# yongjianxu/ompi-release

Measured on AMD Instinct MI355X. Metric: MPI_Allreduce busbw GB/s (1 GiB fp32, np=8) + op/hip reduce HBM GB/s, higher is better.
Workload: dtype f32; 1 GPU; op/hip 3-buff MPI_SUM MPI_FLOAT, 1 GiB per operand (BASELINE configs[1]); count=268435456, bytes_per_operand=1073741824

## Files before the change

### include/mi355x_rt.h

```cpp
#ifndef MI355X_RT_H
#define MI355X_RT_H

#include <stddef.h>
#include <stdint.h>

#include "mi355x_types.h"

#ifdef __cplusplus
extern "C" {
#endif

const char *mi355x_last_error(void);
int mi355x_version(void);
int mi355x_device_count(int *count);
int mi355x_set_device(int dev);
int mi355x_get_device(int *dev);
int mi355x_stream_create(void **stream);
int mi355x_stream_destroy(void *stream);
int mi355x_stream_sync(void *stream);
int mi355x_device_sync(void);
int mi355x_malloc(void **p, size_t bytes);
int mi355x_free(void *p);
int mi355x_host_alloc(void **p, size_t bytes);
int mi355x_host_free(void *p);
// ... 31 lines not shown
int mi355x_comm_rank(const mi355x_comm_t *comm);
int mi355x_comm_size(const mi355x_comm_t *comm);
int mi355x_comm_barrier(mi355x_comm_t *comm);
int mi355x_comm_vote(mi355x_comm_t *comm, int device, int *engine);
int mi355x_comm_last_algorithm(const mi355x_comm_t *comm);
int mi355x_debug_pipe_token(mi355x_comm_t *comm, int acquire);
int mi355x_debug_token(uint64_t dev_uid, const char *name, int op);

enum mi355x_knob {
    MI355X_KNOB_ALLREDUCE_ALG = 1,
    MI355X_KNOB_REDUCE_ALG = 2,
    MI355X_KNOB_REDUCE_SCATTER_ALG = 3,
    MI355X_KNOB_BLOCKS_PER_CU = 4,
    MI355X_KNOB_TIMEOUT_S = 5,
    MI355X_KNOB_PUSH = 6,
    MI355X_KNOB_IPC_MAX_BYTES = 7,
    MI355X_KNOB_STAGE_BYTES = 8,
    MI355X_KNOB_REDUCE_CHAIN_FANOUT = 10,
    MI355X_KNOB_LL_MAX_BYTES = 9,
    MI355X_KNOB_TIME_PHASES = 11,
    MI355X_KNOB_COPY_BLOCK_KIB = 12,
    MI355X_KNOB_PIPE = 13,
    MI355X_KNOB_PIPE_WG_PER_CU = 14,
    MI355X_KNOB_PIPE_CHUNK_KIB = 15,
    MI355X_KNOB_PIPE_WT = 16,
    MI355X_KNOB_ONE_PHASE_MAX_BYTES = 17,
    MI355X_KNOB_PIPE_REFUSED = 18,
    MI355X_KNOB_SVC_MAX_BYTES = 19,
    MI355X_KNOB_SVC_CALLS = 20,
    MI355X_KNOB_SVC_LAUNCHES = 21,
    MI355X_KNOB_SVC_RESIDENT = 22,
    MI355X_KNOB_SVC_PULL_MAX_BYTES = 23,
    MI355X_KNOB_SVC_PULL_COPY_MAX_BYTES = 24,
    MI355X_KNOB_RCACHE_MAX_MAPS = 25,
    MI355X_KNOB_RCACHE_SIZE_LIMIT = 26,
    MI355X_KNOB_PEER_MAPS = 27,
    MI355X_KNOB_RCACHE_EVICTIONS = 28,
    MI355X_KNOB_FLOWS = 29,
    MI355X_KNOB_FLOWS_FAILED = 30,
    MI355X_KNOB_CREATE_US = 31,
    MI355X_KNOB_SELFTEST_US = 32,
    MI355X_KNOB_SVC_OWNER = 33,
    MI355X_KNOB_SVC_CLAIMS = 34,
    MI355X_KNOB_SVC_IDLE_US = 35,
    MI355X_KNOB_SVC_SHRINK_US = 36,
    MI355X_KNOB_SVC_REGROWS = 37,
    MI355X_KNOB_DEV_SETUP = 38,
    MI355X_KNOB_SETUP_US = 39,
    MI355X_KNOB_SELFTEST = 40,
    MI355X_KNOB_PIPE_CALLS = 41,
    MI355X_KNOB_EXPORT_MISMATCHES = 42,
    MI355X_KNOB_SELFTEST_REUSED = 43,
    MI355X_KNOB_NB_ORDER = 44,
    MI355X_KNOB_SCAN_PART_MIN_BYTES = 45
};
enum mi355x_flow {
    MI355X_FLOW_SVC_LL = 1,
    MI355X_FLOW_SVC_PULL = 2,
    MI355X_FLOW_SVC_COPY = 4,
    MI355X_FLOW_SVC_RS = 8,
    MI355X_FLOW_PIPE = 16
};
int mi355x_comm_set(mi355x_comm_t *comm, int knob, long value);
int mi355x_comm_get(const mi355x_comm_t *comm, int knob, long *value);
int mi355x_comm_phase_ms(const mi355x_comm_t *comm, float *phase1_ms, float *phase2_ms);

enum mi355x_coll_id {
    MI355X_COLL_ALLGATHER = 0, MI355X_COLL_ALLREDUCE = 2, MI355X_COLL_BCAST = 7, MI355X_COLL_REDUCE = 11,
    MI355X_COLL_REDUCESCATTER = 12, MI355X_COLL_COUNT = 16
};
typedef struct mi355x_rules mi355x_rules_t;
int mi355x_rules_load(const char *path, mi355x_rules_t **rules);
int mi355x_rules_destroy(mi355x_rules_t *rules);
int mi355x_rules_decide(const mi355x_rules_t *rules, int coll, int comm_size, size_t msg_bytes, int *alg,
                        int *faninout, int *segsize);
int mi355x_comm_set_rules(mi355x_comm_t *comm, const mi355x_rules_t *rules);

int mi355x_allreduce(mi355x_comm_t *comm, const void *sbuf, void *rbuf, size_t count, int type, int op,
                     void *stream);
int mi355x_reduce(mi355x_comm_t *comm, const void *sbuf, void *rbuf, size_t count, int type, int op, int root,
                  void *stream);
int mi355x_reduce_scatter_block(mi355x_comm_t *comm, const void *sbuf, void *rbuf, size_t rcount,
                                int type, int op, void *stream);
int mi355x_reduce_scatter(mi355x_comm_t *comm, const void *sbuf, void *rbuf, const int *rcounts,
                          int type, int op, void *stream);
int mi355x_allgather(mi355x_comm_t *comm, const void *sbuf, void *rbuf, size_t bytes, void *stream);
int mi355x_bcast(mi355x_comm_t *comm, void *buf, size_t bytes, int root, void *stream);

int mi355x_gather(mi355x_comm_t *comm, const void *sbuf, void *rbuf, size_t bytes, int root, void *stream);
int mi355x_gatherv(mi355x_comm_t *comm, const void *sbuf, size_t sbytes, void *rbuf, const size_t *rcounts,
                   const size_t *displs, int root, void *stream);
int mi355x_scatter(mi355x_comm_t *comm, const void *sbuf, void *rbuf, size_t bytes, int root, void *stream);
int mi355x_scatterv(mi355x_comm_t *comm, const void *sbuf, const size_t *scounts, const size_t *displs,
                    void *rbuf, size_t rbytes, int root, void *stream);
int mi355x_allgatherv(mi355x_comm_t *comm, const void *sbuf, size_t sbytes, void *rbuf, const size_t *rcounts,
                      const size_t *displs, void *stream);
int mi355x_alltoall(mi355x_comm_t *comm, const void *sbuf, void *rbuf, size_t bytes, void *stream);
int mi355x_alltoallv(mi355x_comm_t *comm, const void *sbuf, const size_t *scounts, const size_t *sdispls,
                     void *rbuf, const size_t *rcounts, const size_t *rdispls, void *stream);
int mi355x_scan(mi355x_comm_t *comm, const void *sbuf, void *rbuf, size_t count, int type, int op, void *stream);
int mi355x_exscan(mi355x_comm_t *comm, const void *sbuf, void *rbuf, size_t count, int type, int op, void *stream);
int mi355x_scan_part_plan(size_t count, int n, int q, int r, size_t *src_off, size_t *len, size_t *slot_off);

typedef struct mi355x_request mi355x_request_t;
int mi355x_iallreduce(mi355x_comm_t *comm, const void *sbuf, void *rbuf, size_t count, int type, int op,
                      void *stream, mi355x_request_t **req);
// ... 89 lines not shown
```

### ompi-release_amd/__init__.py

```python
from __future__ import annotations

import ctypes
import os
import pathlib

PKG_DIR = pathlib.Path(__file__).resolve().parent
LIB_DIR = pathlib.Path(os.environ["MI355X_LIB_DIR"]) if os.environ.get("MI355X_LIB_DIR") else PKG_DIR / "lib"
REPO_DIR = PKG_DIR.parent

TYPES = [
    "INT8", "UINT8", "INT16", "UINT16", "INT32", "UINT32", "INT64", "UINT64",
    "F_INTEGER", "F_INTEGER1", "F_INTEGER2", "F_INTEGER4", "F_INTEGER8", "F_INTEGER16",
    "FLOAT", "DOUBLE", "F_REAL", "F_REAL2", "F_REAL4", "F_REAL8", "F_REAL16",
    "F_DOUBLE_PRECISION", "LONG_DOUBLE", "F_LOGICAL", "BOOL",
    "C_FLOAT_COMPLEX", "C_DOUBLE_COMPLEX", "C_LONG_DOUBLE_COMPLEX", "BYTE",
    "F_2REAL", "F_2DOUBLE_PRECISION", "F_2INTEGER",
    "FLOAT_INT", "DOUBLE_INT", "LONG_INT", "2INT", "SHORT_INT", "LONG_DOUBLE_INT", "WCHAR",
]
T = {name: i for i, name in enumerate(TYPES)}
OPS = ["NULL", "MAX", "MIN", "SUM", "PROD", "LAND", "BAND", "LOR", "BOR", "LXOR", "BXOR",
       "MAXLOC", "MINLOC", "REPLACE", "NO_OP"]
OP = {name: i for i, name in enumerate(OPS)}

MI355X_SUCCESS = 0
# ... 181 lines not shown

def op_supported(op: int, ty: int) -> bool:
    return bool(rt().mi355x_op_supported(op, ty))


def comm_op_supported(op: int, ty: int) -> bool:
    return bool(rt().mi355x_comm_op_supported(op, ty))


def type_size(ty: int) -> int:
    return int(rt().mi355x_type_size(ty))


def set_threads(threads: int) -> None:
    check(rt().mi355x_op_set_threads(threads), "mi355x_op_set_threads")


def tune(unroll: int = 0, blocks_per_cu: int = 0, nontemporal: int = -2) -> None:
    check(rt().mi355x_op_tune(unroll, blocks_per_cu, nontemporal), "mi355x_op_tune")


def set_mode(mode: int) -> None:
    check(rt().mi355x_op_set_mode(mode), "mi355x_op_set_mode")


def get_mode() -> int:
    return int(rt().mi355x_op_get_mode())


def get_tune() -> tuple[int, int, int]:
    a, b, c = ctypes.c_int(), ctypes.c_int(), ctypes.c_int()
    check(rt().mi355x_op_get_tune(ctypes.byref(a), ctypes.byref(b), ctypes.byref(c)))
    return a.value, b.value, c.value


def scan_part_plan(count: int, n: int, q: int, r: int) -> tuple[int, int, int | None]:
    a, b, c_ = ctypes.c_size_t(), ctypes.c_size_t(), ctypes.c_size_t()
    check(rt().mi355x_scan_part_plan(count, n, q, r, ctypes.byref(a), ctypes.byref(b), ctypes.byref(c_)),
          "mi355x_scan_part_plan")
    return a.value, b.value, None if r == q else c_.value


KNOB = {"ALLREDUCE_ALG": 1, "REDUCE_ALG": 2, "REDUCE_SCATTER_ALG": 3, "BLOCKS_PER_CU": 4, "TIMEOUT_S": 5,
        "PUSH": 6, "IPC_MAX_BYTES": 7, "STAGE_BYTES": 8,
        "LL_MAX_BYTES": 9, "REDUCE_CHAIN_FANOUT": 10, "TIME_PHASES": 11,
        "COPY_BLOCK_KIB": 12, "PIPE": 13, "PIPE_WG_PER_CU": 14, "PIPE_CHUNK_KIB": 15, "PIPE_WT": 16,
        "ONE_PHASE_MAX_BYTES": 17, "PIPE_REFUSED": 18, "SVC_MAX_BYTES": 19, "SVC_CALLS": 20,
        "SVC_LAUNCHES": 21, "SVC_RESIDENT": 22, "SVC_PULL_MAX_BYTES": 23,
        "SVC_PULL_COPY_MAX_BYTES": 24, "RCACHE_MAX_MAPS": 25, "RCACHE_SIZE_LIMIT": 26, "PEER_MAPS": 27,
        "RCACHE_EVICTIONS": 28, "FLOWS": 29, "FLOWS_FAILED": 30, "CREATE_US": 31, "SELFTEST_US": 32,
        "SVC_OWNER": 33, "SVC_CLAIMS": 34, "SVC_IDLE_US": 35,
        "SVC_SHRINK_US": 36, "SVC_REGROWS": 37, "DEV_SETUP": 38, "SETUP_US": 39, "SELFTEST": 40,
        "PIPE_CALLS": 41, "EXPORT_MISMATCHES": 42, "SELFTEST_REUSED": 43, "NB_ORDER": 44,
        "SCAN_PART_MIN_BYTES": 45}
NBC_ALG = {"BINOMIAL": 101, "RING": 102, "CHAIN": 103}
FLOW = {"SVC_LL": 1, "SVC_PULL": 2, "SVC_COPY": 4, "SVC_RS": 8, "PIPE": 16}
COLL = {"ALLGATHER": 0, "ALLREDUCE": 2, "BCAST": 7, "REDUCE": 11, "REDUCESCATTER": 12}
AR_ALG = {"DECISION": 0, "LINEAR": 1, "NONOVERLAPPING": 2, "RECURSIVE_DOUBLING": 3, "RING": 4,
          "RING_SEGMENTED": 5}


class Comm:

    def __init__(self, handle: int):
        self.h = ctypes.c_void_p(handle)

    @classmethod
    def create(cls, key: str, rank: int, size: int, device: int) -> "Comm":
        h = ctypes.c_void_p()
        check(rt().mi355x_comm_create(key.encode(), rank, size, device, ctypes.byref(h)), "mi355x_comm_create")
        return cls(h.value)

    @classmethod
    def loopback(cls, size: int, device: int = 0) -> list["Comm"]:
        arr = (ctypes.c_void_p * size)()
        check(rt().mi355x_comm_create_loopback(size, device, arr), "mi355x_comm_create_loopback")
        return [cls(arr[i]) for i in range(size)]

    def destroy(self) -> None:
        if self.h:
            rt().mi355x_comm_destroy(self.h)
            self.h = ctypes.c_void_p()

    @property
    def rank(self) -> int:
        return rt().mi355x_comm_rank(self.h)

    @property
    def size(self) -> int:
        return rt().mi355x_comm_size(self.h)

    def barrier(self) -> None:
        check(rt().mi355x_comm_barrier(self.h), "mi355x_comm_barrier")

    def vote(self, device: bool) -> bool:
        anyd = ctypes.c_int(0)
        check(rt().mi355x_comm_vote(self.h, 1 if device else 0, ctypes.byref(anyd)), "mi355x_comm_vote")
        return bool(anyd.value)

    def last_algorithm(self) -> int:
        return rt().mi355x_comm_last_algorithm(self.h)

    def debug_pipe_token(self, acquire: bool) -> bool:
        rc = rt().mi355x_debug_pipe_token(self.h, 1 if acquire else 0)
        if rc < 0:
            check(rc, "mi355x_debug_pipe_token")
        return rc == 1
# ... 336 lines not shown
```

### ompi-release_amd/csrc/rt/coll_comm.cpp

```cpp

#include <fcntl.h>
#include <immintrin.h>
#include <poll.h>
#include <sched.h>
#include <signal.h>
#include <sys/mman.h>
#include <sys/socket.h>
#include <sys/stat.h>
#include <sys/un.h>
#include <unistd.h>

#include <algorithm>
#include <array>
#include <atomic>
#include <cerrno>
#include <chrono>
#include <condition_variable>
#include <cstddef>
#include <deque>
#include <functional>
#include <cstdio>
#include <cstdlib>
#include <cstring>
#include <map>
// ... 326 lines not shown
    if (op) return (c->pipe_entry >= 0 || pipe_token_acquire(c)) ? 1 : 0;
    if (c->pipe_entry >= 0) pipe_token_release(c);
    return 0;
}

int mi355x_debug_pipe_token(mi355x_comm_t *c, int acquire)
{
    if (!c) return set_error(MI355X_ERR_ARG, "comm is NULL");
    if (acquire) return pipe_token_acquire(c) ? 1 : 0;
    if (c->pipe_entry >= 0) pipe_token_release(c);
    return 0;
}
static bool svc_limit_visible(const mi355x_comm_t *c)
{
    return c->svc_ok || c->svc_want || (!c->dev_ready && !c->loopback && c->size > 1);
}

int mi355x_comm_get(const mi355x_comm_t *c, int knob, long *value)
{
    if (!c || !value) return set_error(MI355X_ERR_ARG, "NULL argument");
    switch (knob) {
    case MI355X_KNOB_ALLREDUCE_ALG: *value = c->knob_allreduce; break;
    case MI355X_KNOB_REDUCE_ALG: *value = c->knob_reduce; break;
    case MI355X_KNOB_REDUCE_SCATTER_ALG: *value = c->knob_rs; break;
    case MI355X_KNOB_BLOCKS_PER_CU: *value = c->tune.blocks_per_cu; break;
    case MI355X_KNOB_TIMEOUT_S: *value = (long)c->timeout_s; break;
    case MI355X_KNOB_PUSH: *value = c->tune.push; break;
    case MI355X_KNOB_IPC_MAX_BYTES: *value = (long)c->ipc_max; break;
    case MI355X_KNOB_STAGE_BYTES: *value = (long)c->stage_bytes; break;
    case MI355X_KNOB_PIPE_REFUSED: *value = (long)c->pipe_refused; break;
    case MI355X_KNOB_LL_MAX_BYTES: *value = (long)c->ll_max; break;
    case MI355X_KNOB_REDUCE_CHAIN_FANOUT: *value = c->chain_fanout; break;
    case MI355X_KNOB_TIME_PHASES: *value = c->time_phases ? 1 : 0; break;
    case MI355X_KNOB_COPY_BLOCK_KIB: *value = c->tune.copy_block_kib; break;
    case MI355X_KNOB_PIPE: *value = c->pipe_on ? 1 : 0; break;
    case MI355X_KNOB_PIPE_WG_PER_CU: *value = c->tune.pipe_wg_per_cu; break;
    case MI355X_KNOB_PIPE_CHUNK_KIB: *value = c->tune.pipe_chunk_kib; break;
    case MI355X_KNOB_PIPE_WT: *value = c->tune.pipe_wt; break;
    case MI355X_KNOB_ONE_PHASE_MAX_BYTES: *value = (long)c->one_phase_max; break;
    case MI355X_KNOB_SVC_MAX_BYTES: *value = svc_limit_visible(c) ? (long)c->svc_max : 0; break;
    case MI355X_KNOB_SVC_CALLS: *value = (long)c->svc_calls; break;
    case MI355X_KNOB_SVC_LAUNCHES: *value = (long)c->svc_launches; break;
    case MI355X_KNOB_SVC_RESIDENT: *value = c->svcq && svc_resident(c->svcq) ? 1 : 0; break;
    case MI355X_KNOB_SVC_PULL_MAX_BYTES: *value = svc_limit_visible(c) ? (long)c->svc_pull_max : 0; break;
    case MI355X_KNOB_SVC_PULL_COPY_MAX_BYTES: *value = svc_limit_visible(c) ? (long)c->svc_copy_max : 0; break;
    case MI355X_KNOB_FLOWS: *value = (long)c->flows; break;
    case MI355X_KNOB_FLOWS_FAILED: *value = (long)c->flows_failed; break;
    case MI355X_KNOB_CREATE_US: *value = (long)c->create_us; break;
    case MI355X_KNOB_SELFTEST_US: *value = (long)c->selftest_us; break;
    case MI355X_KNOB_SELFTEST_REUSED: *value = (long)c->selftest_reused; break;
    case MI355X_KNOB_DEV_SETUP: *value = c->dev_ready ? 1 : 0; break;
    case MI355X_KNOB_SELFTEST: *value = c->selftest ? 1 : 0; break;
    case MI355X_KNOB_PIPE_CALLS: *value = (long)c->pipe_calls; break;
    case MI355X_KNOB_EXPORT_MISMATCHES: *value = (long)c->export_mismatches; break;
    case MI355X_KNOB_SETUP_US: *value = (long)c->setup_us; break;
    case MI355X_KNOB_SVC_OWNER: *value = c->svc_ok ? 1 : 0; break;
    case MI355X_KNOB_SVC_CLAIMS: *value = (long)c->svc_epoch; break;
    case MI355X_KNOB_SVC_IDLE_US: *value = (long)(c->svc_idle_s * 1e6 + 0.5); break;
    case MI355X_KNOB_SVC_SHRINK_US: *value = (long)(c->svc_shrink_s * 1e6 + 0.5); break;
    case MI355X_KNOB_SVC_REGROWS: *value = (long)c->svc_regrows; break;
    case MI355X_KNOB_RCACHE_MAX_MAPS: *value = (long)c->rcache_max_maps; break;
    case MI355X_KNOB_RCACHE_SIZE_LIMIT: *value = (long)c->rcache_limit; break;
    case MI355X_KNOB_PEER_MAPS: {
        std::lock_guard<std::recursive_mutex> g(const_cast<mi355x_comm *>(c)->reg_mtx);
        *value = (long)peer_map_count(c);
        break;
    }
    case MI355X_KNOB_RCACHE_EVICTIONS: *value = (long)c->rcache_evictions; break;
    case MI355X_KNOB_NB_ORDER: *value = c->nb_order; break;
    case MI355X_KNOB_SCAN_PART_MIN_BYTES: *value = (long)c->scan_part_min; break;
    default: return set_error(MI355X_ERR_ARG, "unknown knob %d", knob);
    }
    return MI355X_SUCCESS;
}

int mi355x_comm_phase_ms(const mi355x_comm_t *c, float *phase1_ms, float *phase2_ms)
{
    if (!c || !phase1_ms || !phase2_ms) return set_error(MI355X_ERR_ARG, "NULL argument");
    *phase1_ms = c->phase_ms[0];
    *phase2_ms = c->phase_ms[1];
    return MI355X_SUCCESS;
}

int mi355x_comm_set(mi355x_comm_t *c, int knob, long value)
{
    if (!c) return set_error(MI355X_ERR_ARG, "comm is NULL");
    if (!c->dev_ready && !c->loopback && c->size > 1) {
        size_t *field = knob == MI355X_KNOB_LL_MAX_BYTES ? &c->ll_max
                        : knob == MI355X_KNOB_SVC_MAX_BYTES ? &c->svc_max
                        : knob == MI355X_KNOB_SVC_PULL_MAX_BYTES ? &c->svc_pull_max
                        : knob == MI355X_KNOB_SVC_PULL_COPY_MAX_BYTES ? &c->svc_copy_max : nullptr;
        if (field) {
            const long hi = (knob == MI355X_KNOB_LL_MAX_BYTES || knob == MI355X_KNOB_SVC_MAX_BYTES) ? (64l << 20) : (1l << 30);
            if (value < 0 || value > hi) return set_error(MI355X_ERR_ARG, "knob %d out of range", knob);
            *field = (size_t)value;
            c->preset.emplace_back(knob, value);
            return MI355X_SUCCESS;
        }
    }
    switch (knob) {
    case MI355X_KNOB_SELFTEST: c->selftest = value != 0; break;
    case MI355X_KNOB_ALLREDUCE_ALG: c->knob_allreduce = (int)value; break;
    case MI355X_KNOB_REDUCE_ALG: c->knob_reduce = (int)value; break;
    case MI355X_KNOB_REDUCE_SCATTER_ALG: c->knob_rs = (int)value; break;
    case MI355X_KNOB_BLOCKS_PER_CU:
        if (value < 1 || value > 1024) return set_error(MI355X_ERR_ARG, "blocks_per_cu out of range");
// ... 162 lines not shown
```

### ompi-release_amd/csrc/rt/coll_pipe.hip

```cpp
#include "coll_internal.hpp"
#include "op_functors.hpp"
#include "rt_internal.hpp"
#include "slot_list.hpp"
#include "stream_core.hpp"

namespace mi355x {

__device__ __forceinline__ __amdgpu_buffer_rsrc_t wt_rsrc(const void *base)
{
    return __builtin_amdgcn_make_buffer_rsrc(const_cast<void *>(base), 0, 0x7fffffff, 0x00020000);
}

template <class F, bool NT, int U, int FC>
__device__ __forceinline__ void fold_body(const PipeArgs &a, typename F::T *dst, size_t v0, size_t nvec, bool wt)
{
    using T = typename F::T;
    using V = Vec16<T>;
    constexpr int EPV = 16 / sizeof(T);
    const size_t t = threadIdx.x, nt = blockDim.x;
    const __amdgpu_buffer_rsrc_t rs = wt_rsrc(dst + v0);
    for (size_t base = t; base < nvec; base += nt * U) {
        V acc[U];
        for (int j0 = 0; j0 < a.n; j0 += FC) {
            V x[FC][U];
            load_chunk<NT, u32x4>(x, a.src, a.order, v0 * sizeof(T), j0, a.n, base, nt, nvec);
            fold_chunk<F, false>(acc, x, j0, a.n, a.role_mask);
        }
#pragma unroll
        for (int u = 0; u < U; ++u) {
            const size_t v = base + (size_t)u * nt;
            if (v < nvec) {
                u32x4 raw;
                __builtin_memcpy(&raw, &acc[u], 16);
                if (wt) __builtin_amdgcn_raw_buffer_store_b128(raw, rs, (unsigned)(v * 16), 0, kSysCoherent);
                else vstore<NT>(dst + v0 + v * EPV, raw);
            }
        }
    }
}

template <class F, bool NT> __device__ void fold_range(const PipeArgs &a, size_t lo, size_t hi, bool wt)
{
    using T = typename F::T;
    constexpr int EPV = 16 / sizeof(T);
    T *dst = reinterpret_cast<T *>(a.dst);
    const size_t t = threadIdx.x, nt = blockDim.x;
    static_assert((sizeof(T) & (sizeof(T) - 1)) == 0 && sizeof(T) <= 16, "the mask below is 16 - sizeof(T)");
    const Split16 sp = split16(hi - lo, sizeof(T), (uintptr_t)(dst + lo) & (16 - sizeof(T)), a.co_fold);
    const size_t head = sp.head, nvec = sp.nvec;
    for (size_t i = lo + t; i < lo + head; i += nt)
        dst[i] = fold_scalar<F, false>(a.src, a.order, a.role_mask, a.n, i);
    const size_t v0 = lo + head;
    if (a.n <= 4)
        fold_body<F, NT, 4, 4>(a, dst, v0, nvec, wt);
    else
        fold_body<F, NT, 2, kFoldChunk>(a, dst, v0, nvec, wt);
    for (size_t i = v0 + nvec * EPV + t; i < hi; i += nt)
        dst[i] = fold_scalar<F, false>(a.src, a.order, a.role_mask, a.n, i);
}

template <bool NT> __device__ void copy_range(char *dst, const char *src, size_t lo, size_t hi, bool co, bool wt)
{
    const size_t t = threadIdx.x, nt = blockDim.x;
    const Split16 sp = split16(hi - lo, 1, (uintptr_t)(dst + lo) & 15, co);
    const size_t head = sp.head, nvec = sp.nvec;
    for (size_t i = lo + t; i < lo + head; i += nt) dst[i] = src[i];
    const size_t b0 = lo + head;
    constexpr int U = 8;
    const __amdgpu_buffer_rsrc_t rs = wt_rsrc(src + b0);
    for (size_t base = t; base < nvec; base += nt * U) {
        u32x4 x[U];
#pragma unroll
        for (int u = 0; u < U; ++u) {
            const size_t v = base + (size_t)u * nt;
            if (v < nvec)
                x[u] = wt ? __builtin_amdgcn_raw_buffer_load_b128(rs, (unsigned)(v * 16), 0, kSysCoherent)
                          : vload<NT, u32x4>(src + b0 + v * 16);
        }
        store_vecs<NT>(dst + b0, x, base, nt, nvec);
    }
    for (size_t i = b0 + nvec * 16 + t; i < hi; i += nt) dst[i] = src[i];
}

__device__ __forceinline__ uint64_t flag_load(const uint64_t *p)
{
    return __hip_atomic_load(p, __ATOMIC_RELAXED, __HIP_MEMORY_SCOPE_SYSTEM);
}

__device__ __forceinline__ uint64_t uniform64(uint64_t v)
{
    const uint32_t lo = __builtin_amdgcn_readfirstlane((uint32_t)v);
    const uint32_t hi = __builtin_amdgcn_readfirstlane((uint32_t)(v >> 32));
    return ((uint64_t)hi << 32) | lo;
}

__device__ __forceinline__ void dbg_store(const PipeArgs &a, int w, uint64_t v)
{
    if (a.dbg) __hip_atomic_store(a.dbg + 4 * blockIdx.x + w, v, __ATOMIC_RELAXED, __HIP_MEMORY_SCOPE_SYSTEM);
}

template <class F, bool NT> __global__ __launch_bounds__(256) void k_pipe_allreduce(PipeArgs a)
{
    using T = typename F::T;
    constexpr size_t esz = sizeof(T);
    __shared__ uint64_t item_s;
    __shared__ uint32_t give_up_s;
    const uint64_t total = (uint64_t)a.nchunks * (uint64_t)a.n;
    for (;;) {
        if (threadIdx.x == 0) item_s = __hip_atomic_fetch_add(a.queue, 1ull, __ATOMIC_RELAXED, __HIP_MEMORY_SCOPE_AGENT) - a.qbase;
        __syncthreads();
        const uint64_t it = uniform64(item_s);
        if (threadIdx.x == 0) dbg_store(a, 0, it);
        if (it >= total) break;
        if (it < a.nchunks) {
            const uint64_t k = it;
            const size_t blen = a.blen[a.me], lo = k * a.chunk, hi = lo + a.chunk < blen ? lo + a.chunk : blen;
            const bool wt = a.wt && a.co_fold && ((uintptr_t)(a.dst + (a.boff[a.me] + lo) * esz) & 15) == 0 &&
                            (((hi - lo) * esz) & 15) == 0;
            if (lo < hi) fold_range<F, NT>(a, a.boff[a.me] + lo, a.boff[a.me] + hi, wt);
            asm volatile("s_waitcnt vmcnt(0)" ::: "memory");
            __syncthreads();
            if (threadIdx.x == 0) {
                if (!wt) __builtin_amdgcn_fence(__ATOMIC_RELEASE, "");
                asm volatile("s_waitcnt vmcnt(0)" ::: "memory");
                for (int q = 0; q < a.n; ++q)
                    if (q != a.me) __hip_atomic_store(a.peer_flag[q] + k, a.seq, __ATOMIC_RELAXED, __HIP_MEMORY_SCOPE_SYSTEM);
                dbg_store(a, 1, 2);
            }
        } else {
            const uint64_t j = it - a.nchunks;
            const uint64_t k = j / (uint64_t)(a.n - 1);
            const int q = (int)((a.me + 1 + (int)(j % (uint64_t)(a.n - 1))) % a.n);
            const size_t blen = a.blen[q], lo = k * a.chunk, hi = lo + a.chunk < blen ? lo + a.chunk : blen;
            const size_t b0 = (a.boff[q] + lo) * esz, b1 = (a.boff[q] + hi) * esz;
            const bool co = (a.co_pull >> q) & 1u;
            const bool wt = a.wt && co && ((uintptr_t)(a.dst + b0) & 15) == 0 && ((b1 - b0) & 15) == 0;
            if (threadIdx.x == 0) {
                uint32_t give_up = 0;
                const uint64_t *f = a.my_flag + (size_t)q * a.kmax + k;
                const uint64_t t0 = __builtin_amdgcn_s_memrealtime();
                unsigned polls = 0;
                while (flag_load(f) < a.seq) {
                    __builtin_amdgcn_s_sleep(2);
                    if ((++polls & 1023u) == 0 &&
                        (__hip_atomic_load(a.err, __ATOMIC_RELAXED, __HIP_MEMORY_SCOPE_SYSTEM) != 0 ||
                         __builtin_amdgcn_s_memrealtime() - t0 > a.timeout_ticks)) {
                        __hip_atomic_store(a.err, 1u, __ATOMIC_RELAXED, __HIP_MEMORY_SCOPE_SYSTEM);
                        give_up = 1;
                        break;
                    }
                }
                if (!wt) __builtin_amdgcn_fence(__ATOMIC_ACQUIRE, "");
                asm volatile("s_waitcnt vmcnt(0)" ::: "memory");
                give_up_s = give_up;
                dbg_store(a, 1, give_up ? 8 : 4);
                dbg_store(a, 3, polls);
            }
            __syncthreads();
            const bool give_up = __builtin_amdgcn_readfirstlane(give_up_s) != 0;
            if (!give_up && lo < hi) copy_range<NT>(a.dst, a.peer_rbuf[q], b0, b1, co, wt);
        }
        __syncthreads();
    }
}

static bool pipe_nt(size_t bytes) { return beyond_mall(2 * bytes); }

template <class F> static int launch_pipe(const PipeArgs &a, unsigned grid, hipStream_t s)
{
    if (pipe_nt((size_t)a.count * sizeof(typename F::T)))
        hipLaunchKernelGGL((k_pipe_allreduce<F, true>), dim3(grid), dim3(256), 0, s, a);
    else
        hipLaunchKernelGGL((k_pipe_allreduce<F, false>), dim3(grid), dim3(256), 0, s, a);
    MI_HIP(hipGetLastError());
    return MI355X_SUCCESS;
}

template <class F> static int occupancy_pipe(size_t count)
{
    int nb = 0;
    hipError_t e = pipe_nt(count * sizeof(typename F::T))
                       ? hipOccupancyMaxActiveBlocksPerMultiprocessor(&nb, k_pipe_allreduce<F, true>, 256, 0)
                       : hipOccupancyMaxActiveBlocksPerMultiprocessor(&nb, k_pipe_allreduce<F, false>, 256, 0);
    return e == hipSuccess && nb > 0 ? nb : 1;
}

struct PipeTable {
    int (*f[MI355X_OP_MAX_][MI355X_T_MAX])(const PipeArgs &, unsigned, hipStream_t) = {};
    int (*occ[MI355X_OP_MAX_][MI355X_T_MAX])(size_t) = {};
    PipeTable()
    {
        for_each_slot([&](auto tag, int op, int ty) {
            using F = typename decltype(tag)::type;
            f[op][ty] = &launch_pipe<F>;
            occ[op][ty] = &occupancy_pipe<F>;
        });
    }
};

static const PipeTable &pipe_table()
{
    static const PipeTable t;
    return t;
}

int launch_pipe_slot(int op, int type, const PipeArgs &a, unsigned grid, hipStream_t s)
{
    const PipeTable &t = pipe_table();
    if (op < 0 || op >= MI355X_OP_MAX_ || type < 0 || type >= MI355X_T_MAX || !t.f[op][type])
        return set_error(MI355X_ERR_UNSUPPORTED, "no pipelined allreduce for op %d type %d", op, type);
    return t.f[op][type](a, grid, s);
}

// ... 9 lines not shown
```

### ompi-release_amd/csrc/rt/coll_pipe_host.cpp

```cpp

#include <fcntl.h>
#include <immintrin.h>
#include <poll.h>
#include <sched.h>
#include <signal.h>
#include <sys/mman.h>
#include <sys/socket.h>
#include <sys/stat.h>
#include <sys/un.h>
#include <unistd.h>

#include <algorithm>
#include <array>
#include <atomic>
#include <cerrno>
#include <chrono>
#include <condition_variable>
#include <cstddef>
#include <deque>
#include <functional>
#include <cstdio>
#include <cstdlib>
#include <cstring>
#include <map>
#include <memory>
#include <mutex>
#include <string>
#include <thread>
#include <vector>

#include "coll_internal.hpp"
#include "coll_sched.hpp"
#include "rt_internal.hpp"
#include "stream_core.hpp"

#include "comm_internal.hpp"

#include "coll_comm_int.hpp"

namespace mi355x {

constexpr size_t kPipeKmax = 1024;
int ensure_pipe(mi355x_comm *c)
{
    if (c->pipe_base) return MI355X_SUCCESS;
    const size_t n = (size_t)c->size;
    const size_t bytes = (n * kPipeKmax * sizeof(uint64_t) + 4095) / 4096 * 4096;
    MI_HIP(hipExtMallocWithFlags((void **)&c->pipe_base, bytes, hipDeviceMallocUncached));
    hipStream_t ss = setup_stream(c);
    MI_HIP(hipMemsetAsync(c->pipe_base, 0, bytes, ss));
    MI_HIP(hipMalloc((void **)&c->pipe_queue, sizeof(uint64_t)));
    MI_HIP(hipMemsetAsync(c->pipe_queue, 0, sizeof(uint64_t), ss));
    if (!c->ll_err) MI_HIP(hipHostMalloc((void **)&c->ll_err, sizeof(uint32_t), hipHostMallocCoherent));
    MI_HIP(hipStreamSynchronize(ss));
    c->pipe_kmax = kPipeKmax;
    c->pipe_qbase = 0;
    c->pipe_seq = 0;
    const void *mine[1] = {c->pipe_base};
    const uint64_t sig[4] = {11, bytes, 0, 0};
    std::vector<std::vector<void *>> P;
    int rc = exchange(c, 1, mine, sig, P, nullptr, true, true);
    if (rc) return rc;
    c->pipe_peer.assign(n, nullptr);
    for (size_t q = 0; q < n; ++q) c->pipe_peer[q] = (char *)P[0][q];
    TRACE(c, "pipe region %zu bytes, %d ranks on this GPU", bytes, c->pipe_share);
    return barrier(c);
}

}

namespace mi355x {

int pipe_allreduce(mi355x_comm *c, int op, int type, const Program &pr,
                          const std::vector<std::vector<void *>> &P, size_t count, hipStream_t s)
{
    if (!c->pipe_base) return set_error(MI355X_ERR_ARG, "pipelined allreduce before its setup");
    int rc = MI355X_SUCCESS;
    const size_t esz = mi355x_type_size(type), n = (size_t)c->size;
    PipeArgs a;
    std::memset(&a, 0, sizeof(a));
    size_t maxlen = 0;
    for (int q = 0; q < c->size; ++q) {
        size_t o, l;
        ring_block(count, c->size, q, &o, &l);
        a.boff[q] = o;
        a.blen[q] = l;
        maxlen = std::max(maxlen, l);
    }
    const size_t vec = 16 / esz;
    size_t chunk = coll_tune().pipe_chunk_kib ? ((size_t)coll_tune().pipe_chunk_kib << 10) / esz
                                              : std::max<size_t>(((size_t)64 << 10) / esz, maxlen / 512);
    if (c->pipe_chunk_override) chunk = c->pipe_chunk_override;
    chunk = std::max(chunk, (maxlen + kPipeKmax - 1) / kPipeKmax);
    chunk = (chunk + vec - 1) / vec * vec;
    const size_t nchunks = std::max<size_t>(1, (maxlen + chunk - 1) / chunk);
    const int me = c->rank;
    for (int q = 0; q < c->size; ++q) {
        a.src[q] = P[0][q];
        a.peer_rbuf[q] = (const char *)P[1][q];
        if (q != me)
            a.peer_flag[q] = reinterpret_cast<uint64_t *>(c->pipe_peer[q]) + (size_t)me * c->pipe_kmax;
    }
    a.dst = (char *)P[1][me];
    a.my_flag = reinterpret_cast<const uint64_t *>(c->pipe_base);
    a.queue = c->pipe_queue;
    a.err = c->ll_err;
    *c->ll_err = 0;
    a.qbase = c->pipe_qbase;
    a.seq = ++c->pipe_seq;
    a.timeout_ticks = (uint64_t)(c->timeout_s * 1e8);
    a.kmax = c->pipe_kmax;
    a.chunk = chunk;
    a.count = count;
    a.nchunks = (uint32_t)nchunks;
    a.n = c->size;
    a.me = me;
    for (size_t j = 0; j < pr.order.size(); ++j) a.order[j] = pr.order[j];
    a.role_mask = pr.role_mask;
    a.wt = coll_tune().pipe_wt;
    const void *fold_ptrs[1 + kMaxRanks] = {a.dst};
    for (int q = 0; q < c->size; ++q) fold_ptrs[1 + q] = a.src[q];
    a.co_fold = co_aligned(esz, fold_ptrs, 1 + c->size);
    for (int q = 0; q < c->size; ++q) {
        const void *const pull_ptrs[] = {a.dst, a.peer_rbuf[q]};
        if (co_aligned(1, pull_ptrs, 2)) a.co_pull |= 1ull << q;
    }
    const uint64_t total = (uint64_t)nchunks * n;
    const int share = std::max(1, c->pipe_share);
    int wpc = coll_tune().pipe_wg_per_cu;
    if (share > 1) wpc = std::min(wpc, pipe_blocks_per_cu(op, type, count));
    uint64_t grid = (uint64_t)std::max(1, wpc * device_cu_count() / share);
    if (share == 1) grid = std::max<uint64_t>(grid, 8);
    if (grid > total) grid = total;
    const bool tp = c->time_phases && c->tev[0];
    if (tp) MI_HIP(hipEventRecord(c->tev[0], s));
    TRACE(c, "pipe launch seq %llu grid %llu chunks %zu x %zu elements qbase %llu co_fold %d co_pull %llx",
          (unsigned long long)a.seq, (unsigned long long)grid, nchunks, chunk, (unsigned long long)a.qbase, a.co_fold,
          (unsigned long long)a.co_pull);
    if (debug_on()) {
        if (!c->pipe_dbg) MI_HIP(hipHostMalloc((void **)&c->pipe_dbg, 4 * 4096 * sizeof(uint64_t), hipHostMallocCoherent));
        std::memset(c->pipe_dbg, 0, 4 * 4096 * sizeof(uint64_t));
        if (grid <= 4096) a.dbg = c->pipe_dbg;
    }
    rc = launch_pipe_slot(op, type, a, (unsigned)grid, s);
    if (rc) return rc;
    if (tp) MI_HIP(hipEventRecord(c->tev[1], s));
    if (a.dbg) {
        const auto t0 = std::chrono::steady_clock::now();
        double next = 2.0;
        while (hipStreamQuery(s) == hipErrorNotReady) {
            usleep(1000);
            const double el = std::chrono::duration<double>(std::chrono::steady_clock::now() - t0).count();
            if (el > next) {
                next += 5.0;
                for (uint64_t g = 0; g < grid; ++g)
                    TRACE(c, "pipe wg %llu: item %lld stage %lld flag %lld polls %lld", (unsigned long long)g,
                          (long long)c->pipe_dbg[4 * g], (long long)c->pipe_dbg[4 * g + 1], (long long)c->pipe_dbg[4 * g + 2],
                          (long long)c->pipe_dbg[4 * g + 3]);
                uint64_t qv = 0;
                TRACE(c, "pipe err word %u", (unsigned)__atomic_load_n(c->ll_err, __ATOMIC_ACQUIRE));
                (void)qv;
            }
        }
    }
    bool gone = false;
    for (unsigned spins = 1; hipStreamQuery(s) == hipErrorNotReady; ++spins) {
        if (spins > 256) sched_yield();
        if (!gone && (spins & 0x3fffu) == 0 && peer_gone(c)) {
            gone = true;
            __atomic_store_n(c->ll_err, 1u, __ATOMIC_RELEASE);
        }
    }
    MI_HIP(hipStreamSynchronize(s));
    if (__atomic_load_n(c->ll_err, __ATOMIC_ACQUIRE)) {
        if (gone) {
            (void)hipMemsetAsync(c->pipe_queue, 0, sizeof(uint64_t), s);
            (void)hipStreamSynchronize(s);
            c->pipe_qbase = 0;
            return MI355X_ERR_PEER;
// ... 71 lines not shown
```

### ompi-release_amd/csrc/rt/comm_internal.hpp

```cpp
#pragma once

#include <unistd.h>

#include <atomic>
#include <condition_variable>
#include <cstdint>
#include <cstdio>
#include <cstdlib>
#include <deque>
#include <functional>
#include <map>
#include <memory>
#include <mutex>
#include <string>
#include <thread>
#include <vector>

#include "coll_internal.hpp"
#include "coll_sched.hpp"
#include "rt_internal.hpp"
#include "svc_queue.hpp"

namespace mi355x {

// ... 238 lines not shown
    mi355x::SvcQueue *svcq = nullptr;
    mi355x::SvcPage *svc_page = nullptr;
    bool svc_page_dev = false;
    uint64_t *svc_host = nullptr;
    int svc_nwg = 16;
    double svc_idle_s = 0.001;
    double svc_shrink_s = 100e-6;
    uint64_t svc_calls = 0, svc_launches = 0, svc_regrows = 0;
    size_t svc_pull_max = (size_t)128 << 10;
    size_t svc_copy_max = (size_t)1 << 20;
    bool svc_rs = true;
    bool svc_keep = false;
    bool svc_want = false;
    bool svc_attached = false;
    bool svc_flows_tested = false;
    int selftest_reused = 0;
    uint64_t svc_epoch = 0;
    uint64_t svc_tries = 0;
    uint64_t svc_retry = 16;
    uint64_t svc_revocations = 0;
    double svc_handover_s = 0.01;
    unsigned flows = 0x1f, flows_failed = 0;
    bool pipe_untested = false;
    size_t pipe_chunk_override = 0;
    bool gated = false;
    uint64_t gate_calls = 0;
    size_t ll_bytes = 0;
    double create_us = 0, selftest_us = 0;
    void *gf_buf = nullptr;
    size_t gf_bytes = 0;
    double gf_used = 0;
    mi355x::CollTune tune = mi355x::coll_tune_default();
    uint64_t use_clock = 0;
    bool dev_ready = false;
    bool selftest = true;
    double setup_us = 0;
    std::vector<std::pair<int, long>> preset;
    bool svc_stuck = false;
    uint64_t *svc_trace = nullptr;
    char *pipe_base = nullptr;
    size_t pipe_kmax = 0;
    std::vector<char *> pipe_peer;
    uint64_t *pipe_queue = nullptr;
    uint64_t pipe_qbase = 0;
    uint64_t pipe_seq = 0;
    int pipe_share = 1;
    size_t one_phase_max = (size_t)1 << 20;
    bool pipe_on = false;
    uint64_t pipe_holder = 0;
    int pipe_token = -1;
    int pipe_entry = -1;
    uint64_t pipe_refused = 0;
    uint64_t pipe_calls = 0;
    std::mutex prog_mtx;
    std::map<int, mi355x::Program> prog_cache;
    bool lat_on = false;
    double lat_acc[4] = {0, 0, 0, 0};
    uint64_t lat_n = 0;
    char *ctrl_dev = nullptr;
    bool ctrl_registered = false;
    uint64_t done_seq = 0;
    uint64_t *pipe_dbg = nullptr;
    std::thread worker;
    std::mutex q_mtx;
    std::condition_variable q_cv;
    std::deque<mi355x_request *> queue;
    bool stop = false;
    int pending = 0;
    hipStream_t nb_stream = nullptr;
    int knob_allreduce = 0, knob_reduce = 0, knob_rs = 0;
    int chain_fanout = mi355x::kDefaultChainFanout;
    const mi355x_rules_t *rules = nullptr;
    int nb_order = 0;
    size_t scan_part_min = mi355x::kScanPartMinDefault;
    int last_alg = -1;
    double timeout_s = mi355x::kDefaultTimeoutS;
    bool time_phases = false;
    hipEvent_t tev[4] = {nullptr, nullptr, nullptr, nullptr};
    float phase_ms[2] = {-1.f, -1.f};
    mi355x::P2P *p2p = nullptr;
    std::recursive_mutex reg_mtx;
};

namespace mi355x {
int barrier(mi355x_comm *c);
int local_handle(mi355x_comm *c, const void *p, BufDesc *d, bool force);
int export_dmabuf(mi355x_comm *c, BufDesc *d, uint64_t peers);
int fd_drain(mi355x_comm *c, bool wait);
constexpr int kOpenRetry = 1;
int map_peer(mi355x_comm *c, int peer, const BufDesc &d, void **out, PeerMap **entry = nullptr, bool coll = true);
size_t peer_map_count(const mi355x_comm *c);
int exchange(mi355x_comm *c, int nbuf, const void *const *mine, const uint64_t sig[4],
             std::vector<std::vector<void *>> &peers, bool *staged = nullptr, bool force = false,
             bool persistent = false);
int finish(mi355x_comm *c, hipStream_t s);
int ensure_scratch(mi355x_comm *c, size_t bytes);
int run_program(int op, int type, const Program &pr, const std::vector<void *> &in,
                const std::vector<void *> &dst, size_t off, size_t len, hipStream_t s);
int check_common(mi355x_comm *c, int op, int type);
void drain(mi355x_comm *c);
int post(mi355x_comm *c, void *stream, std::function<int(hipStream_t)> run, mi355x_request **out);
void p2p_destroy(mi355x_comm *c);
void gate_enter(mi355x_comm *c);
void gate_exit(mi355x_comm *c);
struct CallGate {
    mi355x_comm *c;
// ... 19 lines not shown
```

Before: 6599 GB/s.

## Align pipe chunks to cache lines and use write-through stores on edge elements

```diff
diff --git a/include/mi355x_rt.h b/include/mi355x_rt.h
--- a/include/mi355x_rt.h
+++ b/include/mi355x_rt.h
@@ -107,6 +107,7 @@
     MI355X_KNOB_EXPORT_MISMATCHES = 42,
     MI355X_KNOB_SELFTEST_REUSED = 43,
     MI355X_KNOB_NB_ORDER = 44,
+    MI355X_KNOB_PIPE_FENCED_ITEMS = 46,
     MI355X_KNOB_SCAN_PART_MIN_BYTES = 45
 };
 enum mi355x_flow {
diff --git a/ompi-release_amd/__init__.py b/ompi-release_amd/__init__.py
--- a/ompi-release_amd/__init__.py
+++ b/ompi-release_amd/__init__.py
@@ -257,7 +257,7 @@
         "SVC_OWNER": 33, "SVC_CLAIMS": 34, "SVC_IDLE_US": 35,
         "SVC_SHRINK_US": 36, "SVC_REGROWS": 37, "DEV_SETUP": 38, "SETUP_US": 39, "SELFTEST": 40,
         "PIPE_CALLS": 41, "EXPORT_MISMATCHES": 42, "SELFTEST_REUSED": 43, "NB_ORDER": 44,
-        "SCAN_PART_MIN_BYTES": 45}
+        "SCAN_PART_MIN_BYTES": 45, "PIPE_FENCED_ITEMS": 46}
 NBC_ALG = {"BINOMIAL": 101, "RING": 102, "CHAIN": 103}
 FLOW = {"SVC_LL": 1, "SVC_PULL": 2, "SVC_COPY": 4, "SVC_RS": 8, "PIPE": 16}
 COLL = {"ALLGATHER": 0, "ALLREDUCE": 2, "BCAST": 7, "REDUCE": 11, "REDUCESCATTER": 12}
diff --git a/ompi-release_amd/csrc/rt/coll_comm.cpp b/ompi-release_amd/csrc/rt/coll_comm.cpp
--- a/ompi-release_amd/csrc/rt/coll_comm.cpp
+++ b/ompi-release_amd/csrc/rt/coll_comm.cpp
@@ -402,6 +402,7 @@
     case MI355X_KNOB_DEV_SETUP: *value = c->dev_ready ? 1 : 0; break;
     case MI355X_KNOB_SELFTEST: *value = c->selftest ? 1 : 0; break;
     case MI355X_KNOB_PIPE_CALLS: *value = (long)c->pipe_calls; break;
+    case MI355X_KNOB_PIPE_FENCED_ITEMS: *value = (long)c->pipe_fenced_items; break;
     case MI355X_KNOB_EXPORT_MISMATCHES: *value = (long)c->export_mismatches; break;
     case MI355X_KNOB_SETUP_US: *value = (long)c->setup_us; break;
     case MI355X_KNOB_SVC_OWNER: *value = c->svc_ok ? 1 : 0; break;
diff --git a/ompi-release_amd/csrc/rt/coll_pipe.hip b/ompi-release_amd/csrc/rt/coll_pipe.hip
--- a/ompi-release_amd/csrc/rt/coll_pipe.hip
+++ b/ompi-release_amd/csrc/rt/coll_pipe.hip
@@ -1,5 +1,6 @@
 #include "coll_internal.hpp"
 #include "op_functors.hpp"
+#include "pipe_chunks.hpp"
 #include "rt_internal.hpp"
 #include "slot_list.hpp"
 #include "stream_core.hpp"
@@ -9,6 +10,53 @@
 __device__ __forceinline__ __amdgpu_buffer_rsrc_t wt_rsrc(const void *base)
 {
     return __builtin_amdgcn_make_buffer_rsrc(const_cast<void *>(base), 0, 0x7fffffff, 0x00020000);
+}
+
+typedef unsigned int u32x2 __attribute__((ext_vector_type(2)));
+template <int B> struct EdgeRaw;
+template <> struct EdgeRaw<1> { using type = uint8_t; };
+template <> struct EdgeRaw<2> { using type = uint16_t; };
+template <> struct EdgeRaw<4> { using type = uint32_t; };
+template <> struct EdgeRaw<8> { using type = u32x2; };
+template <> struct EdgeRaw<16> { using type = u32x4; };
+
+template <int B> __device__ __forceinline__ typename EdgeRaw<B>::type wt_load_elem(__amdgpu_buffer_rsrc_t rs, unsigned off)
+{
+    if constexpr (B == 1) return __builtin_amdgcn_raw_buffer_load_b8(rs, off, 0, kSysCoherent);
+    else if constexpr (B == 2) return __builtin_amdgcn_raw_buffer_load_b16(rs, off, 0, kSysCoherent);
+    else if constexpr (B == 4) return __builtin_amdgcn_raw_buffer_load_b32(rs, off, 0, kSysCoherent);
+    else if constexpr (B == 8) return __builtin_amdgcn_raw_buffer_load_b64(rs, off, 0, kSysCoherent);
+    else return __builtin_amdgcn_raw_buffer_load_b128(rs, off, 0, kSysCoherent);
+}
+
+template <int B> __device__ __forceinline__ void wt_store_elem(typename EdgeRaw<B>::type v, __amdgpu_buffer_rsrc_t rs, unsigned off)
+{
+    if constexpr (B == 1) __builtin_amdgcn_raw_buffer_store_b8(v, rs, off, 0, kSysCoherent);
+    else if constexpr (B == 2) __builtin_amdgcn_raw_buffer_store_b16(v, rs, off, 0, kSysCoherent);
+    else if constexpr (B == 4) __builtin_amdgcn_raw_buffer_store_b32(v, rs, off, 0, kSysCoherent);
+    else if constexpr (B == 8) __builtin_amdgcn_raw_buffer_store_b64(v, rs, off, 0, kSysCoherent);
+    else __builtin_amdgcn_raw_buffer_store_b128(v, rs, off, 0, kSysCoherent);
+}
+
+template <class F> __device__ __forceinline__ void fold_edge_wt(const PipeArgs &a, typename F::T *dst, size_t lo, size_t hi)
+{
+    using T = typename F::T;
+    const size_t i = lo + threadIdx.x;
+    if (i < hi) {
+        const T v = fold_scalar<F, false>(a.src, a.order, a.role_mask, a.n, i);
+        typename EdgeRaw<sizeof(T)>::type raw;
+        __builtin_memcpy(&raw, &v, sizeof(T));
+        wt_store_elem<sizeof(T)>(raw, wt_rsrc(dst + lo), (unsigned)(threadIdx.x * sizeof(T)));
+    }
+}
+
+template <int B> __device__ __forceinline__ void copy_edge_wt(char *dst, const char *src, size_t lo, size_t hi)
+{
+    const size_t i = lo + threadIdx.x * B;
+    if (i < hi) {
+        const typename EdgeRaw<B>::type raw = wt_load_elem<B>(wt_rsrc(src + lo), (unsigned)(threadIdx.x * B));
+        __builtin_memcpy(dst + i, &raw, B);
+    }
 }
 
 template <class F, bool NT, int U, int FC>
@@ -48,23 +96,29 @@
     static_assert((sizeof(T) & (sizeof(T) - 1)) == 0 && sizeof(T) <= 16, "the mask below is 16 - sizeof(T)");
     const Split16 sp = split16(hi - lo, sizeof(T), (uintptr_t)(dst + lo) & (16 - sizeof(T)), a.co_fold);
     const size_t head = sp.head, nvec = sp.nvec;
-    for (size_t i = lo + t; i < lo + head; i += nt)
-        dst[i] = fold_scalar<F, false>(a.src, a.order, a.role_mask, a.n, i);
+    if (wt) fold_edge_wt<F>(a, dst, lo, lo + head);
+    else
+        for (size_t i = lo + t; i < lo + head; i += nt)
+            dst[i] = fold_scalar<F, false>(a.src, a.order, a.role_mask, a.n, i);
     const size_t v0 = lo + head;
     if (a.n <= 4)
         fold_body<F, NT, 4, 4>(a, dst, v0, nvec, wt);
     else
         fold_body<F, NT, 2, kFoldChunk>(a, dst, v0, nvec, wt);
-    for (size_t i = v0 + nvec * EPV + t; i < hi; i += nt)
-        dst[i] = fold_scalar<F, false>(a.src, a.order, a.role_mask, a.n, i);
-}
-
-template <bool NT> __device__ void copy_range(char *dst, const char *src, size_t lo, size_t hi, bool co, bool wt)
+    if (wt) fold_edge_wt<F>(a, dst, v0 + nvec * EPV, hi);
+    else
+        for (size_t i = v0 + nvec * EPV + t; i < hi; i += nt)
+            dst[i] = fold_scalar<F, false>(a.src, a.order, a.role_mask, a.n, i);
+}
+
+template <bool NT, int B> __device__ void copy_range(char *dst, const char *src, size_t lo, size_t hi, bool co, bool wt)
 {
     const size_t t = threadIdx.x, nt = blockDim.x;
     const Split16 sp = split16(hi - lo, 1, (uintptr_t)(dst + lo) & 15, co);
     const size_t head = sp.head, nvec = sp.nvec;
-    for (size_t i = lo + t; i < lo + head; i += nt) dst[i] = src[i];
+    if (wt) copy_edge_wt<B>(dst, src, lo, lo + head);
+    else
+        for (size_t i = lo + t; i < lo + head; i += nt) dst[i] = src[i];
     const size_t b0 = lo + head;
     constexpr int U = 8;
     const __amdgpu_buffer_rsrc_t rs = wt_rsrc(src + b0);
@@ -79,7 +133,9 @@
         }
         store_vecs<NT>(dst + b0, x, base, nt, nvec);
     }
-    for (size_t i = b0 + nvec * 16 + t; i < hi; i += nt) dst[i] = src[i];
+    if (wt) copy_edge_wt<B>(dst, src, b0 + nvec * 16, hi);
+    else
+        for (size_t i = b0 + nvec * 16 + t; i < hi; i += nt) dst[i] = src[i];
 }
 
 __device__ __forceinline__ uint64_t flag_load(const uint64_t *p)
@@ -114,10 +170,9 @@
         if (it >= total) break;
         if (it < a.nchunks) {
             const uint64_t k = it;
-            const size_t blen = a.blen[a.me], lo = k * a.chunk, hi = lo + a.chunk < blen ? lo + a.chunk : blen;
-            const bool wt = a.wt && a.co_fold && ((uintptr_t)(a.dst + (a.boff[a.me] + lo) * esz) & 15) == 0 &&
-                            (((hi - lo) * esz) & 15) == 0;
-            if (lo < hi) fold_range<F, NT>(a, a.boff[a.me] + lo, a.boff[a.me] + hi, wt);
+            const PipeRange r = pipe_chunk(a.boff[a.me], a.blen[a.me], a.chunk, esz, k);
+            const bool wt = pipe_item_wt(a.wt, a.co_fold, (uintptr_t)a.dst);
+            if (r.lo < r.hi) fold_range<F, NT>(a, r.lo, r.hi, wt);
             asm volatile("s_waitcnt vmcnt(0)" ::: "memory");
             __syncthreads();
             if (threadIdx.x == 0) {
@@ -131,10 +186,10 @@
             const uint64_t j = it - a.nchunks;
             const uint64_t k = j / (uint64_t)(a.n - 1);
             const int q = (int)((a.me + 1 + (int)(j % (uint64_t)(a.n - 1))) % a.n);
-            const size_t blen = a.blen[q], lo = k * a.chunk, hi = lo + a.chunk < blen ? lo + a.chunk : blen;
-            const size_t b0 = (a.boff[q] + lo) * esz, b1 = (a.boff[q] + hi) * esz;
+            const PipeRange r = pipe_chunk(a.boff[q], a.blen[q], a.chunk, esz, k);
+            const size_t b0 = r.lo * esz, b1 = r.hi * esz;
             const bool co = (a.co_pull >> q) & 1u;
-            const bool wt = a.wt && co && ((uintptr_t)(a.dst + b0) & 15) == 0 && ((b1 - b0) & 15) == 0;
+            const bool wt = pipe_item_wt(a.wt, co, (uintptr_t)a.dst);
             if (threadIdx.x == 0) {
                 uint32_t give_up = 0;
                 const uint64_t *f = a.my_flag + (size_t)q * a.kmax + k;
@@ -158,7 +213,7 @@
             }
             __syncthreads();
             const bool give_up = __builtin_amdgcn_readfirstlane(give_up_s) != 0;
-            if (!give_up && lo < hi) copy_range<NT>(a.dst, a.peer_rbuf[q], b0, b1, co, wt);
+            if (!give_up && b0 < b1) copy_range<NT, (int)esz>(a.dst, a.peer_rbuf[q], b0, b1, co, wt);
         }
         __syncthreads();
     }
diff --git a/ompi-release_amd/csrc/rt/coll_pipe_host.cpp b/ompi-release_amd/csrc/rt/coll_pipe_host.cpp
--- a/ompi-release_amd/csrc/rt/coll_pipe_host.cpp
+++ b/ompi-release_amd/csrc/rt/coll_pipe_host.cpp
@@ -31,6 +31,7 @@
 
 #include "coll_internal.hpp"
 #include "coll_sched.hpp"
+#include "pipe_chunks.hpp"
 #include "rt_internal.hpp"
 #include "stream_core.hpp"
 
@@ -40,7 +41,6 @@
 
 namespace mi355x {
 
-constexpr size_t kPipeKmax = 1024;
 int ensure_pipe(mi355x_comm *c)
 {
     if (c->pipe_base) return MI355X_SUCCESS;
@@ -87,13 +87,12 @@
         a.blen[q] = l;
         maxlen = std::max(maxlen, l);
     }
-    const size_t vec = 16 / esz;
     size_t chunk = coll_tune().pipe_chunk_kib ? ((size_t)coll_tune().pipe_chunk_kib << 10) / esz
                                               : std::max<size_t>(((size_t)64 << 10) / esz, maxlen / 512);
     if (c->pipe_chunk_override) chunk = c->pipe_chunk_override;
-    chunk = std::max(chunk, (maxlen + kPipeKmax - 1) / kPipeKmax);
-    chunk = (chunk + vec - 1) / vec * vec;
-    const size_t nchunks = std::max<size_t>(1, (maxlen + chunk - 1) / chunk);
+    chunk = pipe_chunk_len(chunk, maxlen, esz);
+    size_t nchunks = 1;
+    for (int q = 0; q < c->size; ++q) nchunks = std::max(nchunks, pipe_nchunks(a.boff[q], a.blen[q], chunk, esz));
     const int me = c->rank;
     for (int q = 0; q < c->size; ++q) {
         a.src[q] = P[0][q];
@@ -125,6 +124,11 @@
         const void *const pull_ptrs[] = {a.dst, a.peer_rbuf[q]};
         if (co_aligned(1, pull_ptrs, 2)) a.co_pull |= 1ull << q;
     }
+    c->pipe_fenced_items = 0;
+    for (int q = 0; q < c->size; ++q) {
+        const bool co = q == me ? a.co_fold != 0 : ((a.co_pull >> q) & 1u) != 0;
+        if (!pipe_item_wt(a.wt != 0, co, (uintptr_t)a.dst)) c->pipe_fenced_items += pipe_nchunks(a.boff[q], a.blen[q], chunk, esz);
+    }
     const uint64_t total = (uint64_t)nchunks * n;
     const int share = std::max(1, c->pipe_share);
     int wpc = coll_tune().pipe_wg_per_cu;
diff --git a/ompi-release_amd/csrc/rt/comm_internal.hpp b/ompi-release_amd/csrc/rt/comm_internal.hpp
--- a/ompi-release_amd/csrc/rt/comm_internal.hpp
+++ b/ompi-release_amd/csrc/rt/comm_internal.hpp
@@ -314,6 +314,7 @@
     int pipe_entry = -1;
     uint64_t pipe_refused = 0;
     uint64_t pipe_calls = 0;
+    uint64_t pipe_fenced_items = 0;
     std::mutex prog_mtx;
     std::map<int, mi355x::Program> prog_cache;
     bool lat_on = false;
diff --git a/ompi-release_amd/csrc/rt/pipe_chunks.hpp b/ompi-release_amd/csrc/rt/pipe_chunks.hpp
--- /dev/null
+++ b/ompi-release_amd/csrc/rt/pipe_chunks.hpp
@@ -0,0 +1,50 @@
+#pragma once
+
+#include <cstddef>
+#include <cstdint>
+
+#ifndef MI_HD
+#define MI_HD __host__ __device__ inline
+#endif
+
+namespace mi355x {
+
+constexpr size_t kPipeKmax = 1024;
+constexpr size_t kPipeLine = 128;
+
+MI_HD size_t pipe_chunk_len(size_t want, size_t maxlen, size_t esz)
+{
+    const size_t line = kPipeLine / esz, least = (maxlen + kPipeKmax - 1) / kPipeKmax;
+    if (want < least) want = least;
+    if (want < 1) want = 1;
+    return (want + line - 1) / line * line;
+}
+
+struct PipeRange {
+    size_t lo, hi;
+};
+
+MI_HD PipeRange pipe_chunk(size_t off, size_t len, size_t chunk, size_t esz, size_t k)
+{
+    const size_t line = kPipeLine / esz, end = off + len;
+    const size_t a = (off + line - 1) / line * line;
+    size_t lo = k ? a + k * chunk : off, hi = a + (k + 1) * chunk;
+    if (lo > end) lo = end;
+    if (hi > end) hi = end;
+    return PipeRange{lo, hi};
+}
+
+MI_HD size_t pipe_nchunks(size_t off, size_t len, size_t chunk, size_t esz)
+{
+    const size_t line = kPipeLine / esz;
+    const size_t head = (off + line - 1) / line * line - off;
+    if (len == 0) return 0;
+    return len <= head ? 1 : (len - head + chunk - 1) / chunk;
+}
+
+MI_HD bool pipe_item_wt(bool wt_knob, bool co, uintptr_t dst)
+{
+    return wt_knob && co && (dst & 15) == 0;
+}
+
+}
```

Result: slower. 6286 GB/s (-4.7%).
